# MyrtleSoftware/myrtlespeech

Measured on AMD Instinct MI355X. Metric: audio-sec/s (RTF), DS2 5xBiLSTM-1024 encoder forward + CTC greedy, 80-feature 10 s clips @ batch 32/GPU, higher is better.
Workload: dtype f16x3 (f32 split in fp16 hi+lo, 3 fp16 MFMA passes, f32 acc: LSTM, projections, conv1/2, FC1; FC2/CTC/decode f32)

## Files before the change

### myrtlespeech_amd/csrc/conv_cl.hip

```cpp
#include <algorithm>
#include <type_traits>

#include "common.h"

namespace {

typedef unsigned u32x4 __attribute__((ext_vector_type(4)));
typedef unsigned u32x2 __attribute__((ext_vector_type(2)));
typedef __bf16 bf16x8 __attribute__((ext_vector_type(8)));
typedef _Float16 f16x8 __attribute__((ext_vector_type(8)));

constexpr int CL_F = 2;

struct ClP {
  int N, Cin, Fin, Tin, Cout, Fout, Tout, KF, KT, SF, ST, DF, DT, pad_f, pad_t;
  int KG;
  int PW;
  int co_tiles;
  int act;
  float lo, hi;
  int FP;
};

__device__ __forceinline__ unsigned bf16b(float x) { return (unsigned)__builtin_bit_cast(unsigned short, (__bf16)x); }
__device__ __forceinline__ unsigned f16b(float x) { return (unsigned)__builtin_bit_cast(unsigned short, (_Float16)x); }
__device__ __forceinline__ void split_by_prec(float x, int prec, unsigned& hi, unsigned& lo) {
  if (prec == ms::PREC_F16) { hi = f16b(x); lo = 0u; }
  else if (prec == ms::PREC_F16X3) ms::plane_split<true>(x, hi, lo);
  else ms::plane_split<false>(x, hi, lo);
}

__global__ void conv_cl_pack_kernel(const float* __restrict__ w, unsigned short* __restrict__ packed, int Cout, int Cin,
                                    int KF, int KT, int cout_pad, int prec, const float* __restrict__ scale_word) {
  const int KG = Cin / 8;
  const float wscale = scale_word[0];
  const size_t plane = (size_t)KF * KT * KG * cout_pad * 8;
  for (size_t i = (size_t)blockIdx.x * blockDim.x + threadIdx.x; i < plane; i += (size_t)gridDim.x * blockDim.x) {
    const int e = i & 7;
    const int co = (i >> 3) % cout_pad;
    const int kg = (i / ((size_t)8 * cout_pad)) % KG;
    const int kt = (i / ((size_t)8 * cout_pad * KG)) % KT;
    const int kf = i / ((size_t)8 * cout_pad * KG * KT);
    float x = 0.f;
    if (co < Cout) x = w[(((size_t)co * Cin + kg * 8 + e) * KF + kf) * KT + kt] * wscale;
    unsigned h, l;
    split_by_prec(x, prec, h, l);
    packed[i] = (unsigned short)h;
    packed[plane + i] = (unsigned short)l;
  }
}

template <int P, bool WIN = false, int WF = 1>
__global__ __launch_bounds__(256, 2) void maskconv_cl_kernel(const unsigned short* __restrict__ xh,
                                                             const unsigned short* __restrict__ xl,
                                                             const int32_t* __restrict__ lens,
                                                             const unsigned short* __restrict__ wp,
                                                             const float* __restrict__ bias, float* __restrict__ y, ClP p,
                                                             const float* __restrict__ scale_word) {
  constexpr bool F16 = ms::prec_one_plane(P), HM = P == ms::PREC_F16X3;
  constexpr int WT = 4 / WF;
  constexpr int TT = 32 * WT;
  constexpr int RF = CL_F * WF;
  extern __shared__ __attribute__((aligned(16))) char lds[];
  const int row_bytes = p.KG * p.PW * 16;
  char* Ph = lds;
  char* Pl = lds + RF * row_bytes;
  char* Wh = lds + 2 * RF * row_bytes;
  const int wtap = p.KG * 32 * 16;
  char* Wl = Wh + ((p.KT + 1) / 2) * wtap;

  const int tid = threadIdx.x, lane = tid & 63, wave = tid >> 6;
  const int l31 = lane & 31, half = lane >> 5;
  const int wt = wave % WT, wf = wave / WT;
  const int t0 = blockIdx.x * TT;
  const int fo0 = blockIdx.y * RF;
  const int n = blockIdx.z / p.co_tiles, tile = blockIdx.z % p.co_tiles;
  const int len = lens ? min(lens[n], p.Tin) : p.Tin;
  const int cout_pad = p.co_tiles * 32;
  const size_t wplane = (size_t)p.KF * p.KT * p.KG * cout_pad * 8;

  ms::f32x16 acc[CL_F];
#pragma unroll
  for (int f = 0; f < CL_F; ++f)
#pragma unroll
    for (int r = 0; r < 16; ++r) acc[f][r] = 0.f;

  const int tin0 = t0 * p.ST - p.pad_t;
  const int ngran = p.KG * p.PW;
  const unsigned plane_bytes = WIN ? (unsigned)((size_t)p.N * p.Tin * p.FP * 2) : 0u;
  const __amdgpu_buffer_rsrc_t xh_rsrc = __builtin_amdgcn_make_buffer_rsrc(const_cast<unsigned short*>(xh), 0, plane_bytes, 0x00020000);
  const __amdgpu_buffer_rsrc_t xl_rsrc = __builtin_amdgcn_make_buffer_rsrc(const_cast<unsigned short*>(xl), 0, plane_bytes, 0x00020000);

  for (int kf = 0; kf < p.KF; ++kf) {
    for (int f = 0; f < RF; ++f) {
      const int fin = (fo0 + f) * p.SF - p.pad_f + kf * p.DF;
      const bool frow = (fo0 + f) < p.Fout && (WIN || (fin >= 0 && fin < p.Fin));
      const size_t rbase = ((size_t)n * p.Fin + (frow && !WIN ? fin : 0)) * p.Tin;
      for (int i = tid; i < ngran; i += 256) {
        const int q = i / p.KG, kg = i - q * p.KG;
        const int tin = tin0 + q;
        u32x4 vh = {0u, 0u, 0u, 0u}, vl = {0u, 0u, 0u, 0u};
        if (frow && tin >= 0 && tin < len) {
          if (WIN) {
            const int boff = (int)((((size_t)n * p.Tin + tin) * p.FP + (size_t)(fo0 + f) * p.SF + kg * 8) * 2);
            vh = __builtin_amdgcn_raw_buffer_load_b128(xh_rsrc, boff, 0, 0);
            if (!F16) vl = __builtin_amdgcn_raw_buffer_load_b128(xl_rsrc, boff, 0, 0);
          } else {
            const size_t off = (rbase + tin) * p.Cin + kg * 8;
            vh = *reinterpret_cast<const u32x4*>(xh + off);
            if (!F16) vl = *reinterpret_cast<const u32x4*>(xl + off);
          }
        }
        *reinterpret_cast<u32x4*>(Ph + f * row_bytes + (kg * p.PW + q) * 16) = vh;
        if (!F16) *reinterpret_cast<u32x4*>(Pl + f * row_bytes + (kg * p.PW + q) * 16) = vl;
      }
    }
    const int taps_per_stage = (p.KT + 1) / 2;
    for (int kt0 = 0; kt0 < p.KT; kt0 += taps_per_stage) {
      const int ntap = min(taps_per_stage, p.KT - kt0);
      if (kt0 > 0) __syncthreads();
      {
        const int ng = ntap * p.KG * 32;
        for (int i = tid; i < ng; i += 256) {
          const int co = i & 31, rest = i >> 5;
          const size_t src = ((((size_t)kf * p.KT + kt0) * p.KG + rest) * cout_pad + tile * 32 + co) * 8;
          *reinterpret_cast<u32x4*>(Wh + i * 16) = *reinterpret_cast<const u32x4*>(wp + src);
          if (!F16) *reinterpret_cast<u32x4*>(Wl + i * 16) = *reinterpret_cast<const u32x4*>(wp + wplane + src);
        }
      }
      __syncthreads();
      for (int ktl = 0; ktl < ntap; ++ktl) {
        const int tq = (wt * 32 + l31) * p.ST + (kt0 + ktl) * p.DT;
        for (int s = 0; s < p.KG / 2; ++s) {
          const int kg = 2 * s + half;
          const int woff = ((ktl * p.KG + kg) * 32 + l31) * 16;
          const u32x4 ah = *reinterpret_cast<const u32x4*>(Wh + woff);
          u32x4 al = ah;
          if (!F16) al = *reinterpret_cast<const u32x4*>(Wl + woff);
#pragma unroll
          for (int f = 0; f < CL_F; ++f) {
            const int poff = (wf * CL_F + f) * row_bytes + (kg * p.PW + tq) * 16;
            const u32x4 bh = *reinterpret_cast<const u32x4*>(Ph + poff);
            if (F16) {
              acc[f] = __builtin_amdgcn_mfma_f32_32x32x16_f16(__builtin_bit_cast(f16x8, ah), __builtin_bit_cast(f16x8, bh), acc[f], 0, 0, 0);
            } else {
              const u32x4 bl = *reinterpret_cast<const u32x4*>(Pl + poff);
              acc[f] = ms::mfma_32x32x16<HM>(ah, bh, acc[f]);
              acc[f] = ms::mfma_32x32x16<HM>(al, bh, acc[f]);
              acc[f] = ms::mfma_32x32x16<HM>(ah, bl, acc[f]);
            }
          }
        }
      }
    }
    __syncthreads();
  }

  const int t = t0 + wt * 32 + l31;
  const float winv = scale_word[1];
  if (t < p.Tout) {
#pragma unroll
    for (int f = 0; f < CL_F; ++f) {
      const int fo = fo0 + wf * CL_F + f;
      if (fo >= p.Fout) continue;
#pragma unroll
      for (int r = 0; r < 16; ++r) {
        const int co = tile * 32 + ms::mfma32_row(r, lane);
        if (co < p.Cout) {
          float v = acc[f][r] * winv + (bias ? bias[co] : 0.f);
          if (p.act == MS_ACT_CLAMP) v = fminf(fmaxf(v, p.lo), p.hi);
          y[(((size_t)n * p.Cout + co) * p.Fout + fo) * p.Tout + t] = v;
        }
      }
    }
  }
}


constexpr int SH_RB = 12;
constexpr int SH_KT = 11;

template <int P>
__global__ __launch_bounds__(256, 1) void maskconv_cl_short_kernel(const unsigned short* __restrict__ xh,
                                                                   const unsigned short* __restrict__ xl,
                                                                   const int32_t* __restrict__ lens,
                                                                   const unsigned short* __restrict__ wp,
                                                                   const float* __restrict__ bias, float* __restrict__ y, ClP p,
                                                                   int RB, int RIN, const float* __restrict__ scale_word) {
  constexpr bool F16 = ms::prec_one_plane(P), HM = P == ms::PREC_F16X3;
  const float winv = scale_word[1];
  extern __shared__ __attribute__((aligned(16))) char lds[];
  const int tid = threadIdx.x, lane = tid & 63, wave = __builtin_amdgcn_readfirstlane(tid >> 6);
  const int c16 = lane & 15, q = lane >> 4;
  const int fo0 = blockIdx.x * RB, cb = blockIdx.y, n = blockIdx.z;
  const int PW = p.PW;
  const int row_bytes = PW * 64;
  char* Ph = lds;
  char* Pl = lds + (size_t)RIN * row_bytes;
  const int len = lens ? min(lens[n], p.Tin) : p.Tin;
  const int fin_lo = fo0 * p.SF - p.pad_f;

  for (int i = tid; i < RIN * PW * 4; i += 256) {
    const int kg = i & 3, rq = i >> 2;
    const int r = rq / PW, fq = rq - r * PW;
    const int fin = fin_lo + r, tin = fq - p.pad_t;
    u32x4 vh = {0u, 0u, 0u, 0u}, vl = {0u, 0u, 0u, 0u};
    if (fin >= 0 && fin < p.Fin && tin >= 0 && tin < len) {
      const size_t off = (((size_t)n * p.Fin + fin) * p.Tin + tin) * 32 + kg * 8;
      vh = *reinterpret_cast<const u32x4*>(xh + off);
      if (!F16) vl = *reinterpret_cast<const u32x4*>(xl + off);
    }
    *reinterpret_cast<u32x4*>(Ph + r * row_bytes + fq * 64 + kg * 16) = vh;
    if (!F16) *reinterpret_cast<u32x4*>(Pl + r * row_bytes + fq * 64 + kg * 16) = vl;
  }
  __syncthreads();

  ms::f32x4 acc[SH_RB];
#pragma unroll
  for (int i = 0; i < SH_RB; ++i) acc[i] = ms::f32x4{0.f, 0.f, 0.f, 0.f};
  const int cout_pad = p.co_tiles * 32;
  const size_t wplane = (size_t)p.KF * p.KT * 4 * cout_pad * 8;
  const unsigned short* wa = wp + (size_t)q * cout_pad * 8 + (cb * 16 + c16) * 8;
  const size_t tap_stride = (size_t)4 * cout_pad * 8;
  u32x4 fh[2][SH_KT], fl[2][SH_KT];
  auto load_row = [&](auto set, int kf) {
#pragma unroll
    for (int kt = 0; kt < SH_KT; ++kt)
      if (kt < p.KT) {
        const unsigned short* src = wa + (size_t)(kf * p.KT + kt) * tap_stride;
        fh[set][kt] = *reinterpret_cast<const u32x4*>(src);
        if (!F16) fl[set][kt] = *reinterpret_cast<const u32x4*>(src + wplane);
      }
  };
  auto compute_row = [&](auto set, int kf) {
#pragma unroll
    for (int i = 0; i < SH_RB; ++i) {
      const int fo = fo0 + i;
      const int fin = fo * p.SF - p.pad_f + kf * p.DF;
      if (i < RB && fo < p.Fout && fin >= 0 && fin < p.Fin) {
        const int rbase = (fin - fin_lo) * row_bytes + c16 * 64 + q * 16;
#pragma unroll
        for (int kt = 0; kt < SH_KT; ++kt)
          if (kt < p.KT) {
            const u32x4 bh = *reinterpret_cast<const u32x4*>(Ph + rbase + kt * 64);
            if (F16) {
              acc[i] = __builtin_amdgcn_mfma_f32_16x16x32_f16(__builtin_bit_cast(f16x8, fh[set][kt]), __builtin_bit_cast(f16x8, bh), acc[i], 0, 0, 0);
            } else {
              const u32x4 bl = *reinterpret_cast<const u32x4*>(Pl + rbase + kt * 64);
              acc[i] = ms::mfma_16x16x32<HM>(fh[set][kt], bh, acc[i]);
              acc[i] = ms::mfma_16x16x32<HM>(fl[set][kt], bh, acc[i]);
              acc[i] = ms::mfma_16x16x32<HM>(fh[set][kt], bl, acc[i]);
            }
          }
      }
    }
  };
  constexpr std::integral_constant<int, 0> S0{};
  constexpr std::integral_constant<int, 1> S1{};
  if (wave < p.KF) load_row(S0, wave);
  for (int kf = wave; kf < p.KF; kf += 8) {
    if (kf + 4 < p.KF) load_row(S1, kf + 4);
    compute_row(S0, kf);
    if (kf + 8 < p.KF) load_row(S0, kf + 8);
    if (kf + 4 < p.KF) compute_row(S1, kf + 4);
  }

  __syncthreads();
  ms::f32x4* part = reinterpret_cast<ms::f32x4*>(lds);
#pragma unroll
  for (int i = 0; i < SH_RB; ++i)
    if (i < RB) part[(wave * SH_RB + i) * 64 + lane] = acc[i];
  __syncthreads();
#pragma unroll
  for (int j = 0; j < SH_RB / 4; ++j) {
    const int i = wave + 4 * j, fo = fo0 + i;
    if (i >= RB || fo >= p.Fout) continue;
    ms::f32x4 v = part[(0 * SH_RB + i) * 64 + lane];
#pragma unroll
    for (int w = 1; w < 4; ++w) v += part[(w * SH_RB + i) * 64 + lane];
    if (c16 < p.Tout) {
#pragma unroll
      for (int r = 0; r < 4; ++r) {
        const int co = cb * 16 + 4 * q + r;
        if (co < p.Cout) {
          float o = v[r] * winv + (bias ? bias[co] : 0.f);
          if (p.act == MS_ACT_CLAMP) o = fminf(fmaxf(o, p.lo), p.hi);
          y[(((size_t)n * p.Cout + co) * p.Fout + fo) * p.Tout + c16] = o;
        }
      }
    }
  }
}

int conv_cl_short_plan(const ClP& p, bool f16, int* RB, int* RIN, size_t* lds) {
  static const bool off = getenv("MS_CONV_SHORT") && getenv("MS_CONV_SHORT")[0] == '0';
  if (off || p.Cin != 32 || p.Tout > 16 || p.ST != 1 || p.DT != 1 || p.FP != 0 || p.N > 65535 || p.KT > SH_KT) return 0;
  const int cbs = ms::cdiv(p.Cout, 16);
  int nblk = std::max(1, std::min(ms::cdiv(p.Fout, 4), ms::cdiv(ms::num_cus(), p.N * cbs)));
  while (ms::cdiv(p.Fout, nblk) > SH_RB) ++nblk;
  for (; nblk <= p.Fout; ++nblk) {
    const int rb = ms::cdiv(p.Fout, nblk);
    const int rin = (rb - 1) * p.SF + (p.KF - 1) * p.DF + 1;
    const size_t bytes = std::max((size_t)(f16 ? 1 : 2) * rin * (p.Tout + p.KT - 1) * 64, (size_t)4 * SH_RB * 64 * 16);
    if (bytes <= 156 * 1024) { *RB = rb; *RIN = rin; *lds = bytes; return 1; }
  }
  return 0;
}

__global__ void nchw_to_cl_split_kernel(const float* __restrict__ x, unsigned short* __restrict__ hi,
                                        unsigned short* __restrict__ lo, int C, int F, int T, int prec) {
  __shared__ float tile[32][33];
  const int n = blockIdx.z / F, f = blockIdx.z % F;
  const int t0 = blockIdx.x * 32, c0 = blockIdx.y * 32;
  const int tx = threadIdx.x, ty = threadIdx.y;
  for (int i = ty; i < 32; i += 8) {
    const int c = c0 + i, t = t0 + tx;
    tile[i][tx] = (c < C && t < T) ? x[(((size_t)n * C + c) * F + f) * T + t] : 0.f;
  }
  __syncthreads();
  for (int i = ty; i < 32; i += 8) {
    const int t = t0 + i, c = c0 + tx;
    if (t < T && c < C) {
      const float v = tile[tx][i];
      const size_t o = (((size_t)n * F + f) * T + t) * C + c;
      unsigned h, l;
      split_by_prec(v, prec, h, l);
      hi[o] = (unsigned short)h;
      if (prec != ms::PREC_F16) lo[o] = (unsigned short)l;
    }
  }
}

__global__ void ft_to_tf_split_kernel(const float* __restrict__ x, unsigned short* __restrict__ hi,
                                      unsigned short* __restrict__ lo, int Fin, int T, int FP, int pad, int prec) {
  __shared__ float tile[32][33];
  const int n = blockIdx.z;
  const int t0 = blockIdx.x * 32, j0 = blockIdx.y * 32;
  const int tx = threadIdx.x, ty = threadIdx.y;
  for (int i = ty; i < 32; i += 8) {
    const int fidx = j0 + i - pad, t = t0 + tx;
    tile[i][tx] = (fidx >= 0 && fidx < Fin && t < T) ? x[((size_t)n * Fin + fidx) * T + t] : 0.f;
  }
  __syncthreads();
  for (int i = ty; i < 32; i += 8) {
    const int t = t0 + i, j = j0 + tx;
    if (t < T && j < FP) {
      const float v = tile[tx][i];
      const size_t o = ((size_t)n * T + t) * FP + j;
      unsigned h, l;
      split_by_prec(v, prec, h, l);
      hi[o] = (unsigned short)h;
      if (prec != ms::PREC_F16) lo[o] = (unsigned short)l;
    }
  }
}

__global__ void conv_fwin_pack_kernel(const float* __restrict__ w, unsigned short* __restrict__ packed, int Cout, int KF,
                                      int KT, int KG, int cout_pad, int prec, const float* __restrict__ scale_word) {
  const size_t plane = (size_t)KT * KG * cout_pad * 8;
  const float wscale = scale_word[0];
  for (size_t i = (size_t)blockIdx.x * blockDim.x + threadIdx.x; i < plane; i += (size_t)gridDim.x * blockDim.x) {
    const int e = i & 7;
    const int co = (i >> 3) % cout_pad;
    const int kg = (i / ((size_t)8 * cout_pad)) % KG;
    const int kt = i / ((size_t)8 * cout_pad * KG);
    const int kf = kg * 8 + e;
    float x = 0.f;
    if (co < Cout && kf < KF) x = w[((size_t)co * KF + kf) * KT + kt] * wscale;
    unsigned h, l;
    split_by_prec(x, prec, h, l);
    packed[i] = (unsigned short)h;
    packed[plane + i] = (unsigned short)l;
  }
}

int conv_cl_plan(ClP& p, size_t* lds) {
  const size_t wbytes = (size_t)2 * ((p.KT + 1) / 2) * p.KG * 32 * 16;
  if ((long)p.N * p.co_tiles > 65535) return 0;
  for (int wf : {p.Tout <= 48 ? 4 : 1, 1}) {
    const int tt = 128 / wf, rf = CL_F * wf;
    p.PW = (tt - 1) * p.ST + (p.KT - 1) * p.DT + 1;
    *lds = (size_t)2 * rf * p.KG * p.PW * 16 + wbytes;
    if (*lds <= 160 * 1024 && ms::cdiv(p.Fout, rf) <= 65535) return wf;
  }
  return 0;
}

template <bool WIN>
int conv_cl_launch(const ClP& p, int wf, size_t lds, const unsigned short* xh, const unsigned short* xl, const int32_t* lens,
                   const void* packed_w, const float* bias, float* y, hipStream_t stream, const float* scale_word) {
  static ms::DeviceOnce attr_once;
  if (attr_once.need()) {
#define MS_CL_ATTR(PP)                                                                                                                     \
    MS_HIP(hipFuncSetAttribute((const void*)maskconv_cl_kernel<PP, WIN, 1>, hipFuncAttributeMaxDynamicSharedMemorySize, 160 * 1024));   \
    MS_HIP(hipFuncSetAttribute((const void*)maskconv_cl_kernel<PP, WIN, 4>, hipFuncAttributeMaxDynamicSharedMemorySize, 160 * 1024));
    MS_CL_ATTR(ms::PREC_BF16X3) MS_CL_ATTR(ms::PREC_F16) MS_CL_ATTR(ms::PREC_F16X3)
#undef MS_CL_ATTR
    attr_once.done();
  }
  const int prec = ms::split_mode();
  const int tt = 128 / wf, rf = CL_F * wf;
  dim3 grid(ms::cdiv(p.Tout, tt), ms::cdiv(p.Fout, rf), p.N * p.co_tiles);
  const unsigned short* wq = (const unsigned short*)packed_w;
#define MS_CL_LAUNCH(WF_)                                                                                                             \
  if (prec == ms::PREC_F16) hipLaunchKernelGGL((maskconv_cl_kernel<ms::PREC_F16, WIN, WF_>), grid, dim3(256), lds, stream, xh, xl, lens, wq, bias, y, p, scale_word); \
  else if (prec == ms::PREC_F16X3) hipLaunchKernelGGL((maskconv_cl_kernel<ms::PREC_F16X3, WIN, WF_>), grid, dim3(256), lds, stream, xh, xl, lens, wq, bias, y, p, scale_word); \
  else hipLaunchKernelGGL((maskconv_cl_kernel<ms::PREC_BF16X3, WIN, WF_>), grid, dim3(256), lds, stream, xh, xl, lens, wq, bias, y, p, scale_word);
  if (wf == 4) { MS_CL_LAUNCH(4) } else { MS_CL_LAUNCH(1) }
#undef MS_CL_LAUNCH
  MS_LAUNCH_CHECK();
  return MS_OK;
}

inline int fwin_kfp(int KF) { return ms::cdiv(KF, 16) * 16; }
inline int fwin_fp(int KF, int SF, int Fout) { return ms::cdiv((Fout - 1) * SF + fwin_kfp(KF), 32) * 32; }

}

static size_t fwin_plane_bytes(int Cout, int KF, int KT) {
  return ms::align_up((size_t)2 * KT * (fwin_kfp(KF) / 8) * (ms::cdiv(Cout, 32) * 32) * 8 * sizeof(unsigned short), 256);
}
extern "C" size_t ms_maskconv_fwin_packed_bytes(int Cout, int KF, int KT) {
  if (Cout <= 0 || KF <= 0 || KT <= 0) return 0;
  return fwin_plane_bytes(Cout, KF, KT) + 256;
}

extern "C" int ms_maskconv_fwin_pack(const float* w, void* packed, int Cout, int KF, int KT, void* stream) {
  MS_REQUIRE(w && packed, "null pointer");
  MS_REQUIRE(Cout > 0 && KF > 0 && KT > 0, "bad shape");
  const int cout_pad = ms::cdiv(Cout, 32) * 32, KG = fwin_kfp(KF) / 8;
  const size_t plane = (size_t)KT * KG * cout_pad * 8;
  const int blocks = (int)std::min<size_t>((plane + 255) / 256, 2048);
  float* scale_word = (float*)((char*)packed + fwin_plane_bytes(Cout, KF, KT));
  const int rc = ms::weight_scale_launch(w, (size_t)Cout * KF * KT, scale_word, ms::split_mode(), (hipStream_t)stream);
  if (rc != MS_OK) return rc;
  hipLaunchKernelGGL(conv_fwin_pack_kernel, dim3(blocks), dim3(256), 0, (hipStream_t)stream, w, (unsigned short*)packed, Cout,
                     KF, KT, KG, cout_pad, ms::split_mode(), scale_word);
  MS_LAUNCH_CHECK();
  return MS_OK;
}

extern "C" size_t ms_maskconv_fwin_workspace_bytes(int N, int Tin, int KF, int SF, int Fout) {
  if (N <= 0 || Tin <= 0 || KF <= 0 || SF <= 0 || Fout <= 0) return 0;
  return ms::align_up((size_t)N * Tin * fwin_fp(KF, SF, Fout) * 4, 256);
}

extern "C" int ms_maskconv_fwin_forward(const float* x, const int32_t* lens, const void* packed_w, const float* bias, float* y,
                                        int N, int Fin, int Tin, int Cout, int Fout, int Tout, int KF, int KT, int SF, int ST,
                                        int DT, int pad_f_l, int pad_t_l, int act, float act_lo, float act_hi, void* workspace,
                                        size_t workspace_bytes, void* stream_) {
  ms::ProfScope prof_span(MS_PROF_CONV, (hipStream_t)stream_);
  MS_REQUIRE(x && packed_w && y && workspace, "null pointer");
  MS_REQUIRE(N > 0 && Fin > 0 && Tin > 0 && Cout > 0 && Fout > 0 && Tout > 0, "bad shape");
  MS_REQUIRE(KF > 0 && KT > 0 && SF > 0 && ST > 0 && DT > 0 && pad_f_l >= 0 && pad_t_l >= 0, "bad kernel");
  MS_REQUIRE(SF % 2 == 0, "feature stride must be even (4-byte aligned window loads)");
  MS_REQUIRE(act == MS_ACT_NONE || act == MS_ACT_CLAMP, "bad act");
  if (workspace_bytes < ms_maskconv_fwin_workspace_bytes(N, Tin, KF, SF, Fout)) {
    ms::set_error("ms_maskconv_fwin_forward: workspace too small");
    return MS_ERR_WORKSPACE;
  }
  hipStream_t stream = (hipStream_t)stream_;
  ClP p;
  p.N = N; p.Cin = fwin_kfp(KF); p.Fin = 1; p.Tin = Tin; p.Cout = Cout; p.Fout = Fout; p.Tout = Tout; p.KF = 1; p.KT = KT;
  p.SF = SF; p.ST = ST; p.DF = 1; p.DT = DT; p.pad_f = 0; p.pad_t = pad_t_l; p.KG = p.Cin / 8;
  p.co_tiles = ms::cdiv(Cout, 32);
  p.act = act; p.lo = act_lo; p.hi = act_hi;
  p.FP = fwin_fp(KF, SF, Fout);
  size_t lds = 0;
  const int wf = conv_cl_plan(p, &lds);
  if (wf == 0 || (size_t)N * Tin * p.FP * 2 >= ((size_t)1 << 31)) {
    ms::set_error("ms_maskconv_fwin_forward: shape outside the LDS / grid budget");
    return MS_ERR_UNSUPPORTED;
  }
  unsigned short* xh = (unsigned short*)workspace;
  unsigned short* xl = xh + (size_t)N * Tin * p.FP;
  const int prec = ms::split_mode();
  const bool f16 = prec == ms::PREC_F16;
  hipLaunchKernelGGL(ft_to_tf_split_kernel, dim3(ms::cdiv(Tin, 32), ms::cdiv(p.FP, 32), N), dim3(32, 8), 0, stream, x, xh, xl,
                     Fin, Tin, p.FP, pad_f_l, prec);
  MS_LAUNCH_CHECK();
  return conv_cl_launch<true>(p, wf, lds, xh, xl, lens, packed_w, bias, y, stream,
                              (const float*)((const char*)packed_w + fwin_plane_bytes(Cout, KF, KT)));
}

static size_t cl_plane_bytes(int Cout, int Cin, int KF, int KT) {
  return ms::align_up((size_t)2 * KF * KT * (Cin / 8) * (ms::cdiv(Cout, 32) * 32) * 8 * sizeof(unsigned short), 256);
}
extern "C" size_t ms_maskconv_cl_packed_bytes(int Cout, int Cin, int KF, int KT) {
  if (Cout <= 0 || Cin <= 0 || Cin % 16 || KF <= 0 || KT <= 0) return 0;
  return cl_plane_bytes(Cout, Cin, KF, KT) + 256;
}

extern "C" int ms_maskconv_cl_pack(const float* w, void* packed, int Cout, int Cin, int KF, int KT, void* stream) {
  MS_REQUIRE(w && packed, "null pointer");
  MS_REQUIRE(Cout > 0 && Cin > 0 && Cin % 16 == 0 && KF > 0 && KT > 0, "bad shape (Cin must be a multiple of 16)");
  const int cout_pad = ms::cdiv(Cout, 32) * 32;
  const size_t plane = (size_t)KF * KT * (Cin / 8) * cout_pad * 8;
  const int blocks = (int)std::min<size_t>((plane + 255) / 256, 2048);
  float* scale_word = (float*)((char*)packed + cl_plane_bytes(Cout, Cin, KF, KT));
  const int rc = ms::weight_scale_launch(w, (size_t)Cout * Cin * KF * KT, scale_word, ms::split_mode(), (hipStream_t)stream);
  if (rc != MS_OK) return rc;
  hipLaunchKernelGGL(conv_cl_pack_kernel, dim3(blocks), dim3(256), 0, (hipStream_t)stream, w, (unsigned short*)packed, Cout,
                     Cin, KF, KT, cout_pad, ms::split_mode(), scale_word);
  MS_LAUNCH_CHECK();
  return MS_OK;
}

extern "C" size_t ms_maskconv_cl_workspace_bytes(int N, int Cin, int Fin, int Tin) {
  if (N <= 0 || Cin <= 0 || Fin <= 0 || Tin <= 0) return 0;
  return ms::align_up((size_t)N * Cin * Fin * Tin * 4, 256);
}

extern "C" int ms_maskconv_cl_forward(const float* x, const int32_t* lens, const void* packed_w, const float* bias, float* y,
                                      int N, int Cin, int Fin, int Tin, int Cout, int Fout, int Tout, int KF, int KT,
                                      int SF, int ST, int DF, int DT, int pad_f_l, int pad_t_l, int act, float act_lo,
                                      float act_hi, void* workspace, size_t workspace_bytes, void* stream_) {
  ms::ProfScope prof_span(MS_PROF_CONV, (hipStream_t)stream_);
  MS_REQUIRE(x && packed_w && y && workspace, "null pointer");
  MS_REQUIRE(N > 0 && Cin > 0 && Cin % 16 == 0 && Fin > 0 && Tin > 0 && Cout > 0 && Fout > 0 && Tout > 0, "bad shape");
  MS_REQUIRE(KF > 0 && KT > 0 && SF > 0 && ST > 0 && DF > 0 && DT > 0 && pad_f_l >= 0 && pad_t_l >= 0, "bad kernel");
  MS_REQUIRE(act == MS_ACT_NONE || act == MS_ACT_CLAMP, "bad act");
  if (workspace_bytes < ms_maskconv_cl_workspace_bytes(N, Cin, Fin, Tin)) {
    ms::set_error("ms_maskconv_cl_forward: workspace too small");
    return MS_ERR_WORKSPACE;
  }
  hipStream_t stream = (hipStream_t)stream_;
  ClP p;
  p.N = N; p.Cin = Cin; p.Fin = Fin; p.Tin = Tin; p.Cout = Cout; p.Fout = Fout; p.Tout = Tout; p.KF = KF; p.KT = KT;
  p.SF = SF; p.ST = ST; p.DF = DF; p.DT = DT; p.pad_f = pad_f_l; p.pad_t = pad_t_l; p.KG = Cin / 8;
  p.co_tiles = ms::cdiv(Cout, 32);
  p.act = act; p.lo = act_lo; p.hi = act_hi;
  p.FP = 0;
  size_t lds = 0;
  const int wf = conv_cl_plan(p, &lds);
  if (wf == 0) {
    ms::set_error("ms_maskconv_cl_forward: shape outside the LDS / grid budget");
    return MS_ERR_UNSUPPORTED;
  }
  const float* scale_word = (const float*)((const char*)packed_w + cl_plane_bytes(Cout, Cin, KF, KT));
  unsigned short* xh = (unsigned short*)workspace;
  unsigned short* xl = xh + (size_t)N * Cin * Fin * Tin;
  MS_REQUIRE(N * Fin <= 65535, "N*Fin exceeds grid limits");
  const int prec = ms::split_mode();
  const bool f16 = prec == ms::PREC_F16;
  hipLaunchKernelGGL(nchw_to_cl_split_kernel, dim3(ms::cdiv(Tin, 32), ms::cdiv(Cin, 32), N * Fin), dim3(32, 8), 0, stream, x,
                     xh, xl, Cin, Fin, Tin, prec);
  MS_LAUNCH_CHECK();
  {
    int RB = 0, RIN = 0;
    size_t slds = 0;
    if (conv_cl_short_plan(p, f16, &RB, &RIN, &slds)) {
      static ms::DeviceOnce attr_once;
      if (attr_once.need()) {
        MS_HIP(hipFuncSetAttribute((const void*)maskconv_cl_short_kernel<ms::PREC_BF16X3>, hipFuncAttributeMaxDynamicSharedMemorySize, 160 * 1024));
        MS_HIP(hipFuncSetAttribute((const void*)maskconv_cl_short_kernel<ms::PREC_F16>, hipFuncAttributeMaxDynamicSharedMemorySize, 160 * 1024));
        MS_HIP(hipFuncSetAttribute((const void*)maskconv_cl_short_kernel<ms::PREC_F16X3>, hipFuncAttributeMaxDynamicSharedMemorySize, 160 * 1024));
        attr_once.done();
      }
      ClP ps = p;
      ps.PW = Tout + KT - 1;
      const dim3 grid(ms::cdiv(Fout, RB), ms::cdiv(Cout, 16), N);
      const unsigned short* wq = (const unsigned short*)packed_w;
      auto kern = prec == ms::PREC_F16 ? maskconv_cl_short_kernel<ms::PREC_F16>
                  : prec == ms::PREC_F16X3 ? maskconv_cl_short_kernel<ms::PREC_F16X3> : maskconv_cl_short_kernel<ms::PREC_BF16X3>;
      hipLaunchKernelGGL(kern, grid, dim3(256), slds, stream, xh, xl, lens, wq, bias, y, ps, RB, RIN, scale_word);
      MS_LAUNCH_CHECK();
      return MS_OK;
    }
  }
  return conv_cl_launch<false>(p, wf, lds, xh, xl, lens, packed_w, bias, y, stream, scale_word);
}
```

Measured before the change: 26950.

## Add double-buffered long-time conv kernel for Cin=32, KT=11 layers

Adds a specialized channels-last masked convolution kernel for the second DS2 conv layer (Cin 32, time kernel 11, long sequences). It covers 128 output time steps by 2 frequency rows per block. Global-to-LDS staging is double-buffered across the frequency-tap loop using buffer loads with out-of-range zero fill. Within each tap, LDS-to-register loads are software-pipelined against MFMA issue using sched barriers. This is meant to replace the generic conv_cl path and hide memory latency. In exchange it uses large LDS (up to 160 KB, one block per CU) and a lot of register pressure.

Result: no change. 26940, median of 6 (-0.0%).

```diff
diff --git a/myrtlespeech_amd/csrc/conv_cl.hip b/myrtlespeech_amd/csrc/conv_cl.hip
--- a/myrtlespeech_amd/csrc/conv_cl.hip
+++ b/myrtlespeech_amd/csrc/conv_cl.hip
@@ -307,6 +307,204 @@
   return 0;
 }
 
+constexpr int LG_KG = 4;
+constexpr int LG_XI = 6;
+constexpr int LG_KT = 11;
+constexpr int LG_WI = (LG_KT * LG_KG * 32 + 255) / 256;
+
+template <int P>
+__global__ __launch_bounds__(256, 1) void maskconv_cl_long_kernel(const unsigned short* __restrict__ xh,
+                                                                  const unsigned short* __restrict__ xl,
+                                                                  const int32_t* __restrict__ lens,
+                                                                  const unsigned short* __restrict__ wp,
+                                                                  const float* __restrict__ bias, float* __restrict__ y, ClP p,
+                                                                  const float* __restrict__ scale_word) {
+  constexpr bool F16 = ms::prec_one_plane(P), HM = P == ms::PREC_F16X3;
+  constexpr int NPL = F16 ? 1 : 2;
+  constexpr int KG = LG_KG, KT = LG_KT;
+  extern __shared__ __attribute__((aligned(16))) char lds[];
+  const int row_bytes = KG * p.PW * 16;
+  const int xbytes = CL_F * row_bytes;
+  const int wbytes = KT * KG * 32 * 16;
+  const int stage_bytes = NPL * (xbytes + wbytes);
+
+  const int tid = threadIdx.x, lane = tid & 63, wave = tid >> 6;
+  const int l31 = lane & 31, half = lane >> 5;
+  const int t0 = blockIdx.x * 128;
+  const int fo0 = blockIdx.y * CL_F;
+  const int n = blockIdx.z / p.co_tiles, tile = blockIdx.z % p.co_tiles;
+  const int len = lens ? min(lens[n], p.Tin) : p.Tin;
+  const int cout_pad = p.co_tiles * 32;
+  const size_t wplane = (size_t)p.KF * KT * KG * cout_pad * 8;
+  const int tin0 = t0 * p.ST - p.pad_t;
+  const int ngran = KG * p.PW;
+  const int nx = CL_F * ngran, nw = KT * KG * 32;
+
+  const unsigned plane_bytes = (unsigned)((size_t)p.N * p.Fin * p.Tin * KG * 16);
+  const __amdgpu_buffer_rsrc_t xh_rsrc = __builtin_amdgcn_make_buffer_rsrc(const_cast<unsigned short*>(xh), 0, plane_bytes, 0x00020000);
+  const __amdgpu_buffer_rsrc_t xl_rsrc = __builtin_amdgcn_make_buffer_rsrc(const_cast<unsigned short*>(xl), 0, plane_bytes, 0x00020000);
+
+  u32x4 gxh[LG_XI], gxl[LG_XI], gwh[LG_WI], gwl[LG_WI];
+  auto fetch = [&](int kf) {
+#pragma unroll
+    for (int j = 0; j < LG_XI; ++j) {
+      const int i = tid + 256 * j;
+      const int f = i / ngran, r = i - f * ngran;
+      const int q = r >> 2, kg = r & 3;
+      const int fin = (fo0 + f) * p.SF - p.pad_f + kf * p.DF;
+      const int tin = tin0 + q;
+      const bool ok = i < nx && fo0 + f < p.Fout && fin >= 0 && fin < p.Fin && tin >= 0 && tin < len;
+      const unsigned boff = ok ? (unsigned)(((((size_t)n * p.Fin + fin) * p.Tin + tin) * KG + kg) * 16) : 0x7ffffff0u;
+      gxh[j] = __builtin_amdgcn_raw_buffer_load_b128(xh_rsrc, boff, 0, 0);
+      if (!F16) gxl[j] = __builtin_amdgcn_raw_buffer_load_b128(xl_rsrc, boff, 0, 0);
+    }
+#pragma unroll
+    for (int j = 0; j < LG_WI; ++j) {
+      const int i = tid + 256 * j;
+      if (i < nw) {
+        const int co = i & 31, rest = i >> 5;
+        const size_t src = (((size_t)kf * KT * KG + rest) * cout_pad + tile * 32 + co) * 8;
+        gwh[j] = *reinterpret_cast<const u32x4*>(wp + src);
+        if (!F16) gwl[j] = *reinterpret_cast<const u32x4*>(wp + wplane + src);
+      }
+    }
+  };
+  auto store = [&](char* st) {
+#pragma unroll
+    for (int j = 0; j < LG_XI; ++j) {
+      const int i = tid + 256 * j;
+      if (i < nx) {
+        const int f = i / ngran, r = i - f * ngran;
+        const int off = f * row_bytes + ((r & 3) * p.PW + (r >> 2)) * 16;
+        *reinterpret_cast<u32x4*>(st + off) = gxh[j];
+        if (!F16) *reinterpret_cast<u32x4*>(st + xbytes + off) = gxl[j];
+      }
+    }
+#pragma unroll
+    for (int j = 0; j < LG_WI; ++j) {
+      const int i = tid + 256 * j;
+      if (i < nw) {
+        *reinterpret_cast<u32x4*>(st + NPL * xbytes + i * 16) = gwh[j];
+        if (!F16) *reinterpret_cast<u32x4*>(st + NPL * xbytes + wbytes + i * 16) = gwl[j];
+      }
+    }
+  };
+
+  ms::f32x16 acc[CL_F];
+#pragma unroll
+  for (int f = 0; f < CL_F; ++f)
+#pragma unroll
+    for (int r = 0; r < 16; ++r) acc[f][r] = 0.f;
+
+  auto compute = [&](auto mask, const char* st) {
+    constexpr int M = decltype(mask)::value;
+    const char* X = st;
+    const char* W = st + NPL * xbytes;
+    u32x4 a[2][2][2], b[2][2][CL_F][2];
+    auto load = [&](auto set, int kt) {
+      constexpr int S = decltype(set)::value;
+      const int tq = (wave * 32 + l31) * p.ST + kt * p.DT;
+#pragma unroll
+      for (int s = 0; s < 2; ++s) {
+        const int kg = 2 * s + half;
+        const int woff = ((kt * KG + kg) * 32 + l31) * 16;
+        a[S][s][0] = *reinterpret_cast<const u32x4*>(W + woff);
+        if (!F16) a[S][s][1] = *reinterpret_cast<const u32x4*>(W + wbytes + woff);
+#pragma unroll
+        for (int f = 0; f < CL_F; ++f)
+          if (M >> f & 1) {
+            const int poff = f * row_bytes + (kg * p.PW + tq) * 16;
+            b[S][s][f][0] = *reinterpret_cast<const u32x4*>(X + poff);
+            if (!F16) b[S][s][f][1] = *reinterpret_cast<const u32x4*>(X + xbytes + poff);
+          }
+      }
+    };
+    auto mma = [&](auto set) {
+      constexpr int S = decltype(set)::value;
+#pragma unroll
+      for (int s = 0; s < 2; ++s)
+#pragma unroll
+        for (int f = 0; f < CL_F; ++f)
+          if (M >> f & 1) {
+            if (F16) {
+              acc[f] = __builtin_amdgcn_mfma_f32_32x32x16_f16(__builtin_bit_cast(f16x8, a[S][s][0]), __builtin_bit_cast(f16x8, b[S][s][f][0]), acc[f], 0, 0, 0);
+            } else {
+              acc[f] = ms::mfma_32x32x16<HM>(a[S][s][0], b[S][s][f][0], acc[f]);
+              acc[f] = ms::mfma_32x32x16<HM>(a[S][s][1], b[S][s][f][0], acc[f]);
+              acc[f] = ms::mfma_32x32x16<HM>(a[S][s][0], b[S][s][f][1], acc[f]);
+            }
+          }
+    };
+    constexpr std::integral_constant<int, 0> S0{};
+    constexpr std::integral_constant<int, 1> S1{};
+    load(S0, 0);
+#pragma unroll
+    for (int kt = 0; kt < KT; kt += 2) {
+      if (kt + 1 < KT) load(S1, kt + 1);
+      __builtin_amdgcn_sched_barrier(0);
+      mma(S0);
+      __builtin_amdgcn_sched_barrier(0);
+      if (kt + 2 < KT) load(S0, kt + 2);
+      __builtin_amdgcn_sched_barrier(0);
+      if (kt + 1 < KT) mma(S1);
+      __builtin_amdgcn_sched_barrier(0);
+    }
+  };
+
+  fetch(0);
+  store(lds);
+  __syncthreads();
+  for (int kf = 0; kf < p.KF; ++kf) {
+    const char* st = lds + (kf & 1) * stage_bytes;
+    if (kf + 1 < p.KF) fetch(kf + 1);
+    int m = 0;
+#pragma unroll
+    for (int f = 0; f < CL_F; ++f) {
+      const int fin = (fo0 + f) * p.SF - p.pad_f + kf * p.DF;
+      if (fo0 + f < p.Fout && fin >= 0 && fin < p.Fin) m |= 1 << f;
+    }
+    static_assert(CL_F == 2, "row masks below");
+    if (m == 3) compute(std::integral_constant<int, 3>{}, st);
+    else if (m == 1) compute(std::integral_constant<int, 1>{}, st);
+    else if (m == 2) compute(std::integral_constant<int, 2>{}, st);
+    if (kf + 1 < p.KF) store(lds + ((kf + 1) & 1) * stage_bytes);
+    __syncthreads();
+  }
+
+  const int t = t0 + wave * 32 + l31;
+  const float winv = scale_word[1];
+  if (t < p.Tout) {
+#pragma unroll
+    for (int f = 0; f < CL_F; ++f) {
+      const int fo = fo0 + f;
+      if (fo >= p.Fout) continue;
+#pragma unroll
+      for (int r = 0; r < 16; ++r) {
+        const int co = tile * 32 + ms::mfma32_row(r, lane);
+        if (co < p.Cout) {
+          float v = acc[f][r] * winv + (bias ? bias[co] : 0.f);
+          if (p.act == MS_ACT_CLAMP) v = fminf(fmaxf(v, p.lo), p.hi);
+          y[(((size_t)n * p.Cout + co) * p.Fout + fo) * p.Tout + t] = v;
+        }
+      }
+    }
+  }
+}
+
+int conv_cl_long_plan(ClP& p, bool f16, size_t* lds) {
+  static const bool off = getenv("MS_CONV_LONG") && getenv("MS_CONV_LONG")[0] == '0';
+  if (off || p.Cin != LG_KG * 8 || p.KT != LG_KT || p.FP != 0 || p.Tout <= 48) return 0;
+  if ((long)p.N * p.co_tiles > 65535 || ms::cdiv(p.Fout, CL_F) > 65535) return 0;
+  if ((size_t)p.N * p.Fin * p.Tin * LG_KG * 16 > ((size_t)1 << 30)) return 0;
+  const int pw = 127 * p.ST + (LG_KT - 1) * p.DT + 1;
+  if (CL_F * LG_KG * pw > LG_XI * 256) return 0;
+  const size_t bytes = (size_t)2 * (f16 ? 1 : 2) * (CL_F * LG_KG * pw * 16 + LG_KT * LG_KG * 32 * 16);
+  if (bytes > 160 * 1024) return 0;
+  p.PW = pw;
+  *lds = bytes;
+  return 1;
+}
+
 __global__ void nchw_to_cl_split_kernel(const float* __restrict__ x, unsigned short* __restrict__ hi,
                                         unsigned short* __restrict__ lo, int C, int F, int T, int prec) {
   __shared__ float tile[32][33];
@@ -568,5 +766,25 @@
       return MS_OK;
     }
   }
+  {
+    ClP pl = p;
+    size_t llds = 0;
+    if (conv_cl_long_plan(pl, f16, &llds)) {
+      static ms::DeviceOnce attr_once;
+      if (attr_once.need()) {
+        MS_HIP(hipFuncSetAttribute((const void*)maskconv_cl_long_kernel<ms::PREC_BF16X3>, hipFuncAttributeMaxDynamicSharedMemorySize, 160 * 1024));
+        MS_HIP(hipFuncSetAttribute((const void*)maskconv_cl_long_kernel<ms::PREC_F16>, hipFuncAttributeMaxDynamicSharedMemorySize, 160 * 1024));
+        MS_HIP(hipFuncSetAttribute((const void*)maskconv_cl_long_kernel<ms::PREC_F16X3>, hipFuncAttributeMaxDynamicSharedMemorySize, 160 * 1024));
+        attr_once.done();
+      }
+      const dim3 grid(ms::cdiv(Tout, 128), ms::cdiv(Fout, CL_F), N * pl.co_tiles);
+      const unsigned short* wq = (const unsigned short*)packed_w;
+      auto kern = prec == ms::PREC_F16 ? maskconv_cl_long_kernel<ms::PREC_F16>
+                  : prec == ms::PREC_F16X3 ? maskconv_cl_long_kernel<ms::PREC_F16X3> : maskconv_cl_long_kernel<ms::PREC_BF16X3>;
+      hipLaunchKernelGGL(kern, grid, dim3(256), llds, stream, xh, xl, lens, wq, bias, y, pl, scale_word);
+      MS_LAUNCH_CHECK();
+      return MS_OK;
+    }
+  }
   return conv_cl_launch<false>(p, wf, lds, xh, xl, lens, packed_w, bias, y, stream, scale_word);
 }
```
